# lpiccinelli-eth/UniDepth

Hardware: NVIDIA H100
Metric: images/sec UniDepthV2.infer ViT-L/14 480x640 (higher is better)
Workload: dtype f16 operands, f32 accumulate/residual

## Files before the change

unidepth_b200/csrc/attention.cu:

```cuda
#include "common.h"
#include "ptx.cuh"

namespace udb {

constexpr int AT_BQ = 128;
constexpr int AT_BK = 128;
constexpr int AT_STAGES = 3;
constexpr int AT_THREADS = 288;

struct AttnArgs {
  __half* out;
  int seq_q, seq_k, n_kv_tiles;
  int ldo, o_col0;
  int q_col0, k_col0, v_col0;
  float scale_log2;
};

__device__ __forceinline__ float ex2(float x) {
  float y;
  asm("ex2.approx.ftz.f32 %0, %1;" : "=f"(y) : "f"(x));
  return y;
}

template <int HD>
__global__ void __launch_bounds__(AT_THREADS, 1)
attn_fwd_kernel(const __grid_constant__ CUtensorMap tmQ, const __grid_constant__ CUtensorMap tmK,
                const __grid_constant__ CUtensorMap tmV, const AttnArgs p) {
  static_assert(HD == 64, "head_dim 64 only");
  constexpr int kQBytes = AT_BQ * HD * 2;
  constexpr int kKBytes = AT_BK * HD * 2;
  constexpr int NS = AT_STAGES;
  extern __shared__ __align__(1024) uint8_t smem[];
  uint8_t* sQ = smem;
  uint8_t* sK = sQ + kQBytes;
  uint8_t* sV = sK + NS * kKBytes;
  uint64_t* bars = reinterpret_cast<uint64_t*>(sV + NS * kKBytes);
  uint64_t* q_full = bars;
  uint64_t* k_full = bars + 1;
  uint64_t* v_full = k_full + NS;
  uint64_t* k_empty = v_full + NS;
  uint64_t* v_empty = k_empty + NS;

  const int warp = threadIdx.x >> 5;
  const int lane = threadIdx.x & 31;
  const int q0 = blockIdx.x * AT_BQ;
  const int head = blockIdx.y;
  const int b = blockIdx.z;
  const int n_tiles = p.n_kv_tiles;
  pdl_launch_dependents();

  if (threadIdx.x == 0) {
    if (smem_u32(smem) & 1023) __trap();
    prefetch_tmap(&tmQ);
    prefetch_tmap(&tmK);
    prefetch_tmap(&tmV);
    mbar_init(q_full, 1);
    for (int i = 0; i < NS; ++i) {
      mbar_init(&k_full[i], 1);
      mbar_init(&v_full[i], 1);
      mbar_init(&k_empty[i], 8);
      mbar_init(&v_empty[i], 8);
    }
    fence_barrier_init();
  }
  __syncthreads();
  pdl_wait();

  if (warp == 8) {
    const bool leader = elect_one();
    if (leader) {
      mbar_arrive_expect_tx(q_full, kQBytes);
      tma_load_3d(sQ, &tmQ, q_full, p.q_col0 + head * HD, q0, b);
    }
    __syncwarp();
    int st = 0;
    uint32_t ph = 1;
    for (int j = 0; j < n_tiles; ++j) {
      mbar_wait(&k_empty[st], ph);
      if (leader) {
        mbar_arrive_expect_tx(&k_full[st], kKBytes);
        tma_load_3d(sK + st * kKBytes, &tmK, &k_full[st], p.k_col0 + head * HD, j * AT_BK, b);
      }
      __syncwarp();
      mbar_wait(&v_empty[st], ph);
      if (leader) {
        mbar_arrive_expect_tx(&v_full[st], kKBytes);
        tma_load_3d(sV + st * kKBytes, &tmV, &v_full[st], p.v_col0 + head * HD, j * AT_BK, b);
      }
      __syncwarp();
      if (++st == NS) { st = 0; ph ^= 1; }
    }
    return;
  }

  const int wg = warp >> 2, wq = warp & 3;
  const int cq = 2 * (lane & 3);
  const float sc = p.scale_log2;
  const uint64_t dq = gmma_desc_sw128(smem_u32(sQ + wg * 64 * 128), 16, 1024);
  float o[HD / 2];
#pragma unroll
  for (int i = 0; i < HD / 2; ++i) o[i] = 0.f;
  float m_run[2] = {-INFINITY, -INFINITY}, l_run[2] = {0.f, 0.f};
  mbar_wait(q_full, 0);
  int st = 0;
  uint32_t ph = 0;
  for (int j = 0; j < n_tiles; ++j) {
    float s[AT_BK / 2];
    mbar_wait(&k_full[st], ph);
    {
      const uint64_t dk = gmma_desc_sw128(smem_u32(sK + st * kKBytes), 16, 1024);
      wgmma_fence();
#pragma unroll
      for (int k = 0; k < HD / 16; ++k) wgmma_ss_n128(s, dq + 2 * k, dk + 2 * k, k != 0 ? 1u : 0u);
      wgmma_commit();
      wgmma_wait<0>();
      wgmma_fence_regs(s);
    }
    if (lane == 0) mbar_arrive(&k_empty[st]);
    const int kv_left = p.seq_k - j * AT_BK;
    if (kv_left < AT_BK) {
#pragma unroll
      for (int i = 0; i < AT_BK / 2; ++i)
        if (8 * (i >> 2) + cq + (i & 1) >= kv_left) s[i] = -INFINITY;
    }
#pragma unroll
    for (int h = 0; h < 2; ++h) {
      float mx = -INFINITY;
#pragma unroll
      for (int jj = 0; jj < AT_BK / 8; ++jj) mx = fmaxf(mx, fmaxf(s[4 * jj + 2 * h], s[4 * jj + 2 * h + 1]));
      mx = fmaxf(mx, __shfl_xor_sync(0xffffffffu, mx, 1));
      mx = fmaxf(mx, __shfl_xor_sync(0xffffffffu, mx, 2));
      const float m_new = fmaxf(m_run[h], mx * sc);
      const float alpha = ex2(m_run[h] - m_new);
      m_run[h] = m_new;
      float ls = 0.f;
#pragma unroll
      for (int jj = 0; jj < AT_BK / 8; ++jj) {
        const float e0 = ex2(fmaf(s[4 * jj + 2 * h], sc, -m_new));
        const float e1 = ex2(fmaf(s[4 * jj + 2 * h + 1], sc, -m_new));
        s[4 * jj + 2 * h] = e0;
        s[4 * jj + 2 * h + 1] = e1;
        ls += e0 + e1;
      }
      l_run[h] = fmaf(l_run[h], alpha, ls);
#pragma unroll
      for (int jj = 0; jj < HD / 8; ++jj) {
        o[4 * jj + 2 * h] *= alpha;
        o[4 * jj + 2 * h + 1] *= alpha;
      }
    }
    uint32_t pa[AT_BK / 16][4];
#pragma unroll
    for (int kk = 0; kk < AT_BK / 16; ++kk)
#pragma unroll
      for (int r = 0; r < 4; ++r) pa[kk][r] = pack_half2(s[8 * kk + 2 * r], s[8 * kk + 2 * r + 1]);
    mbar_wait(&v_full[st], ph);
    {
      const uint64_t dv = gmma_desc_sw128(smem_u32(sV + st * kKBytes), 1024, 1024);
      wgmma_fence();
#pragma unroll
      for (int kk = 0; kk < AT_BK / 16; ++kk) wgmma_rs_n64_tb(o, pa[kk], dv + (uint64_t)(kk * 2048 >> 4), 1u);
      wgmma_commit();
      wgmma_wait<0>();
      wgmma_fence_regs(o);
    }
    if (lane == 0) mbar_arrive(&v_empty[st]);
    if (++st == NS) { st = 0; ph ^= 1; }
  }
#pragma unroll
  for (int h = 0; h < 2; ++h) {
    float l = l_run[h];
    l += __shfl_xor_sync(0xffffffffu, l, 1);
    l += __shfl_xor_sync(0xffffffffu, l, 2);
    const float inv = 1.0f / l;
    const int q = q0 + 64 * wg + 16 * wq + (lane >> 2) + 8 * h;
    if (q < p.seq_q) {
      __half* op = p.out + ((long long)b * p.seq_q + q) * p.ldo + p.o_col0 + head * HD + cq;
#pragma unroll
      for (int jj = 0; jj < HD / 8; ++jj)
        *reinterpret_cast<uint32_t*>(op + 8 * jj) = pack_half2(o[4 * jj + 2 * h] * inv, o[4 * jj + 2 * h + 1] * inv);
    }
  }
}

constexpr int SP_T = 64;
constexpr int SP_P = 65;
constexpr int SP_SMEM = (4 * SP_T * SP_P + 3 * SP_T) * 4;

__global__ void __launch_bounds__(256) attn_split_f32_kernel(const udb_attn_t a) {
  extern __shared__ float sp_smem[];
  float* Qs = sp_smem;
  float* Ks = Qs + SP_T * SP_P;
  float* Vs = Ks + SP_T * SP_P;
  float* Ps = Vs + SP_T * SP_P;
  float* m_s = Ps + SP_T * SP_P;
  float* l_s = m_s + SP_T;
  float* al_s = l_s + SP_T;
  const int t = threadIdx.x, ty = t >> 4, tx = t & 15;
  const int q0 = blockIdx.x * SP_T, h = blockIdx.y, b = blockIdx.z;
  const __half* qp = reinterpret_cast<const __half*>(a.q);
  const __half* kp = reinterpret_cast<const __half*>(a.k);
  const __half* vp = reinterpret_cast<const __half*>(a.v);
  auto ld = [](const __half* base, long long off, int lo_off) {
    return __half2float(base[off]) + (lo_off ? __half2float(base[off + lo_off]) : 0.f);
  };
  for (int i = t; i < SP_T * SP_T; i += 256) {
    const int r = i >> 6, d = i & 63;
    const int sq = q0 + r;
    Qs[r * SP_P + d] = sq < a.seq_q ? ld(qp, ((long long)b * a.seq_q + sq) * a.ldq + a.q_col0 + h * 64 + d, a.lo_off_q) * a.scale : 0.f;
  }
  if (t < SP_T) { m_s[t] = -INFINITY; l_s[t] = 0.f; }
  float O[4][4];
#pragma unroll
  for (int i = 0; i < 4; ++i)
#pragma unroll
    for (int j = 0; j < 4; ++j) O[i][j] = 0.f;
  const int n_kt = (a.seq_k + SP_T - 1) / SP_T;
  for (int kt = 0; kt < n_kt; ++kt) {
    __syncthreads();
    for (int i = t; i < SP_T * SP_T; i += 256) {
      const int r = i >> 6, d = i & 63;
      const int sk = kt * SP_T + r;
      const bool ok = sk < a.seq_k;
      const long long row = (long long)b * a.seq_k + sk;
      Ks[r * SP_P + d] = ok ? ld(kp, row * a.ldk + a.k_col0 + h * 64 + d, a.lo_off_k) : 0.f;
      Vs[r * SP_P + d] = ok ? ld(vp, row * a.ldv + a.v_col0 + h * 64 + d, a.lo_off_v) : 0.f;
    }
    __syncthreads();
    float S[4][4];
#pragma unroll
    for (int i = 0; i < 4; ++i)
#pragma unroll
      for (int j = 0; j < 4; ++j) S[i][j] = 0.f;
    for (int d = 0; d < 64; ++d) {
      float qv[4], kv[4];
#pragma unroll
      for (int i = 0; i < 4; ++i) qv[i] = Qs[(ty + 16 * i) * SP_P + d];
#pragma unroll
      for (int j = 0; j < 4; ++j) kv[j] = Ks[(tx + 16 * j) * SP_P + d];
#pragma unroll
      for (int i = 0; i < 4; ++i)
#pragma unroll
        for (int j = 0; j < 4; ++j) S[i][j] = fmaf(qv[i], kv[j], S[i][j]);
    }
#pragma unroll
    for (int i = 0; i < 4; ++i)
#pragma unroll
      for (int j = 0; j < 4; ++j) {
        const int c = tx + 16 * j;
        Ps[(ty + 16 * i) * SP_P + c] = (kt * SP_T + c < a.seq_k) ? S[i][j] : -INFINITY;
      }
    __syncthreads();
    {
      const int r = t >> 2, part = t & 3;
      float* pr = Ps + r * SP_P + part * 16;
      float mx = -INFINITY;
#pragma unroll
      for (int c = 0; c < 16; ++c) mx = fmaxf(mx, pr[c]);
      mx = fmaxf(mx, __shfl_xor_sync(0xffffffffu, mx, 1));
      mx = fmaxf(mx, __shfl_xor_sync(0xffffffffu, mx, 2));
      const float m_old = m_s[r];
      const float m_new = fmaxf(m_old, mx);
      float sum = 0.f;
#pragma unroll
      for (int c = 0; c < 16; ++c) {
        const float pv = expf(pr[c] - m_new);
        pr[c] = pv;
        sum += pv;
      }
      sum += __shfl_xor_sync(0xffffffffu, sum, 1);
      sum += __shfl_xor_sync(0xffffffffu, sum, 2);
      __syncwarp();
      if (part == 0) {
        const float al = expf(m_old - m_new);
        al_s[r] = al;
        m_s[r] = m_new;
        l_s[r] = l_s[r] * al + sum;
      }
    }
    __syncthreads();
#pragma unroll
    for (int i = 0; i < 4; ++i) {
      const float al = al_s[ty + 16 * i];
#pragma unroll
      for (int j = 0; j < 4; ++j) O[i][j] *= al;
    }
    for (int c = 0; c < SP_T; ++c) {
      float pv[4], vv[4];
#pragma unroll
      for (int i = 0; i < 4; ++i) pv[i] = Ps[(ty + 16 * i) * SP_P + c];
#pragma unroll
      for (int j = 0; j < 4; ++j) vv[j] = Vs[c * SP_P + tx + 16 * j];
#pragma unroll
      for (int i = 0; i < 4; ++i)
#pragma unroll
        for (int j = 0; j < 4; ++j) O[i][j] = fmaf(pv[i], vv[j], O[i][j]);
    }
  }
  __half* op = reinterpret_cast<__half*>(a.out);
#pragma unroll
  for (int i = 0; i < 4; ++i) {
    const int r = ty + 16 * i;
    const int sq = q0 + r;
    if (sq >= a.seq_q) continue;
    const float inv = 1.0f / l_s[r];
#pragma unroll
    for (int j = 0; j < 4; ++j) {
      const float v = O[i][j] * inv;
      const long long off = ((long long)b * a.seq_q + sq) * a.ldo + a.o_col0 + h * 64 + tx + 16 * j;
      const __half hi = __float2half_rn(v);
      op[off] = hi;
      if (a.lo_off_o) op[off + a.lo_off_o] = __float2half_rn(v - __half2float(hi));
    }
  }
}

}

extern "C" int udb_attention_f16(const udb_attn_t* a, void* stream) {
  using namespace udb;
  if (a->head_dim != 64) { set_error("udb_attention_f16: head_dim %d unsupported (64 only)", a->head_dim); return 1; }
  if ((a->ldq | a->ldk | a->ldv | a->ldo) % 8) { set_error("udb_attention_f16: leading dims must be multiples of 8"); return 1; }
  if (a->split) {
    static std::atomic<uint64_t> sp_mask{0};
    if (first_on_device(sp_mask)) {
      cudaError_t e = cudaFuncSetAttribute(attn_split_f32_kernel, cudaFuncAttributeMaxDynamicSharedMemorySize, SP_SMEM);
      if (e != cudaSuccess) { set_error("attention(split): cudaFuncSetAttribute: %s", cudaGetErrorString(e)); return 1; }
    }
    dim3 grid((a->seq_q + SP_T - 1) / SP_T, a->heads, a->B);
    attn_split_f32_kernel<<<grid, 256, SP_SMEM, reinterpret_cast<cudaStream_t>(stream)>>>(*a);
    return check_launch("attn_split_f32_kernel");
  }
  constexpr int HD = 64;
  CUtensorMap tq, tk, tv;
  const uint32_t box_q[3] = {HD, AT_BQ, 1};
  const uint32_t box_kv[3] = {HD, AT_BK, 1};
  {
    const uint64_t dims[3] = {(uint64_t)a->ldq, (uint64_t)a->seq_q, (uint64_t)a->B};
    const uint64_t str[2] = {(uint64_t)a->ldq * 2, (uint64_t)a->seq_q * a->ldq * 2};
    if (make_tmap_f16(&tq, a->q, 3, dims, str, box_q, true)) return 1;
  }
  {
    const uint64_t dims[3] = {(uint64_t)a->ldk, (uint64_t)a->seq_k, (uint64_t)a->B};
    const uint64_t str[2] = {(uint64_t)a->ldk * 2, (uint64_t)a->seq_k * a->ldk * 2};
    if (make_tmap_f16(&tk, a->k, 3, dims, str, box_kv, true)) return 1;
  }
  {
    const uint64_t dims[3] = {(uint64_t)a->ldv, (uint64_t)a->seq_k, (uint64_t)a->B};
    const uint64_t str[2] = {(uint64_t)a->ldv * 2, (uint64_t)a->seq_k * a->ldv * 2};
    if (make_tmap_f16(&tv, a->v, 3, dims, str, box_kv, true)) return 1;
  }
  AttnArgs p{};
  p.out = reinterpret_cast<__half*>(a->out);
  p.seq_q = a->seq_q; p.seq_k = a->seq_k;
  p.n_kv_tiles = (a->seq_k + AT_BK - 1) / AT_BK;
  p.ldo = a->ldo; p.o_col0 = a->o_col0;
  p.q_col0 = a->q_col0; p.k_col0 = a->k_col0; p.v_col0 = a->v_col0;
  p.scale_log2 = a->scale * 1.4426950408889634f;
  dim3 grid((a->seq_q + AT_BQ - 1) / AT_BQ, a->heads, a->B);
  note_work(4.0 * a->B * a->heads * (double)a->seq_q * a->seq_k * HD, 2.0 * a->B * a->heads * HD * (2.0 * a->seq_q + 2.0 * a->seq_k));
  constexpr int smem_bytes = 16384 + 2 * AT_STAGES * (AT_BK * 128) + 256;
  static std::atomic<uint64_t> attr_mask{0};
  if (first_on_device(attr_mask)) {
    cudaError_t ea = cudaFuncSetAttribute(attn_fwd_kernel<HD>, cudaFuncAttributeMaxDynamicSharedMemorySize, smem_bytes);
    if (ea != cudaSuccess) { set_error("attention: cudaFuncSetAttribute: %s", cudaGetErrorString(ea)); return 1; }
  }
  cudaError_t e = launch_ex(attn_fwd_kernel<HD>, grid, dim3(AT_THREADS), smem_bytes, reinterpret_cast<cudaStream_t>(stream), 1,
                            tq, tk, tv, p);
  if (e != cudaSuccess) { set_error("attn_fwd_kernel launch: %s", cudaGetErrorString(e)); return 1; }
  return check_launch("attn_fwd_kernel");
}
```

unidepth_b200/csrc/ptx.cuh:

```cuda
#pragma once
#include <cuda_fp16.h>
#include <cuda_runtime.h>
#include <stdint.h>
#include <stdio.h>

namespace udb {

__device__ __forceinline__ uint32_t smem_u32(const void* p) {
  return static_cast<uint32_t>(__cvta_generic_to_shared(p));
}

__device__ __forceinline__ bool elect_one() {
  uint32_t pred = 0;
  asm volatile(
      "{\n\t"
      ".reg .b32 rx;\n\t"
      ".reg .pred px;\n\t"
      "elect.sync rx|px, 0xffffffff;\n\t"
      "selp.b32 %0, 1, 0, px;\n\t"
      "}\n"
      : "=r"(pred));
  return pred != 0;
}

__device__ __forceinline__ void pdl_launch_dependents() {
  asm volatile("griddepcontrol.launch_dependents;" ::: "memory");
}
__device__ __forceinline__ void pdl_wait() { asm volatile("griddepcontrol.wait;" ::: "memory"); }

__device__ __forceinline__ void mbar_init(uint64_t* bar, uint32_t count) {
  asm volatile("mbarrier.init.shared::cta.b64 [%0], %1;" ::"r"(smem_u32(bar)), "r"(count));
}
__device__ __forceinline__ void fence_barrier_init() {
  asm volatile("fence.mbarrier_init.release.cluster;" ::: "memory");
}
__device__ __forceinline__ void mbar_arrive(uint64_t* bar) {
  asm volatile("mbarrier.arrive.shared::cta.b64 _, [%0];" ::"r"(smem_u32(bar)) : "memory");
}
__device__ __forceinline__ void mbar_arrive_expect_tx(uint64_t* bar, uint32_t bytes) {
  asm volatile("mbarrier.arrive.expect_tx.shared::cta.b64 _, [%0], %1;" ::"r"(smem_u32(bar)),
               "r"(bytes)
               : "memory");
}
__device__ __forceinline__ bool mbar_try_wait(uint64_t* bar, uint32_t parity) {
  uint32_t ok;
  asm volatile(
      "{\n\t"
      ".reg .pred p;\n\t"
      "mbarrier.try_wait.parity.shared::cta.b64 p, [%1], %2, %3;\n\t"
      "selp.b32 %0, 1, 0, p;\n\t"
      "}\n"
      : "=r"(ok)
      : "r"(smem_u32(bar)), "r"(parity), "r"(20000u)
      : "memory");
  return ok != 0;
}
#ifndef UDB_SPIN_LIMIT
#define UDB_SPIN_LIMIT (1u << 22)
#endif
__device__ __forceinline__ void mbar_wait(uint64_t* bar, uint32_t parity) {
  if (mbar_try_wait(bar, parity)) return;
  uint32_t spins = 0;
  while (!mbar_try_wait(bar, parity)) {
    if (++spins > UDB_SPIN_LIMIT) __trap();
  }
}

__device__ __forceinline__ void fence_proxy_async_smem() {
  asm volatile("fence.proxy.async.shared::cta;" ::: "memory");
}

__device__ __forceinline__ void prefetch_tmap(const void* tmap) {
  asm volatile("prefetch.tensormap [%0];" ::"l"(reinterpret_cast<uint64_t>(tmap)) : "memory");
}
__device__ __forceinline__ void tma_load_2d(void* smem_dst, const void* tmap, uint64_t* bar, int c0,
                                            int c1) {
  asm volatile(
      "cp.async.bulk.tensor.2d.shared::cluster.global.mbarrier::complete_tx::bytes"
      " [%0], [%1, {%3, %4}], [%2];" ::"r"(smem_u32(smem_dst)),
      "l"(reinterpret_cast<uint64_t>(tmap)), "r"(smem_u32(bar)), "r"(c0), "r"(c1)
      : "memory");
}
__device__ __forceinline__ void tma_load_3d(void* smem_dst, const void* tmap, uint64_t* bar, int c0,
                                            int c1, int c2) {
  asm volatile(
      "cp.async.bulk.tensor.3d.shared::cluster.global.mbarrier::complete_tx::bytes"
      " [%0], [%1, {%3, %4, %5}], [%2];" ::"r"(smem_u32(smem_dst)),
      "l"(reinterpret_cast<uint64_t>(tmap)), "r"(smem_u32(bar)), "r"(c0), "r"(c1), "r"(c2)
      : "memory");
}
__device__ __forceinline__ void tma_load_4d(void* smem_dst, const void* tmap, uint64_t* bar, int c0,
                                            int c1, int c2, int c3) {
  asm volatile(
      "cp.async.bulk.tensor.4d.shared::cluster.global.mbarrier::complete_tx::bytes"
      " [%0], [%1, {%3, %4, %5, %6}], [%2];" ::"r"(smem_u32(smem_dst)),
      "l"(reinterpret_cast<uint64_t>(tmap)), "r"(smem_u32(bar)), "r"(c0), "r"(c1), "r"(c2), "r"(c3)
      : "memory");
}


__device__ __forceinline__ void wgmma_fence() { asm volatile("wgmma.fence.sync.aligned;" ::: "memory"); }
__device__ __forceinline__ void wgmma_commit() { asm volatile("wgmma.commit_group.sync.aligned;" ::: "memory"); }
template <int N>
__device__ __forceinline__ void wgmma_wait() {
  asm volatile("wgmma.wait_group.sync.aligned %0;" ::"n"(N) : "memory");
}
template <int R>
__device__ __forceinline__ void wgmma_fence_regs(float (&d)[R]) {
#pragma unroll
  for (int i = 0; i < R; ++i) asm volatile("" : "+f"(d[i])::"memory");
}
template <uint32_t R>
__device__ __forceinline__ void setmaxnreg_inc() { asm volatile("setmaxnreg.inc.sync.aligned.u32 %0;" ::"n"(R)); }
template <uint32_t R>
__device__ __forceinline__ void setmaxnreg_dec() { asm volatile("setmaxnreg.dec.sync.aligned.u32 %0;" ::"n"(R)); }
__device__ __forceinline__ void bar_sync(int id, int threads) {
  asm volatile("bar.sync %0, %1;" ::"r"(id), "r"(threads) : "memory");
}

__device__ __forceinline__ uint64_t gmma_desc_sw128(uint32_t smem_addr, uint32_t lbo_bytes, uint32_t sbo_bytes) {
  uint64_t d = 0;
  d |= static_cast<uint64_t>((smem_addr & 0x3FFFF) >> 4);
  d |= static_cast<uint64_t>((lbo_bytes >> 4) & 0x3FFF) << 16;
  d |= static_cast<uint64_t>((sbo_bytes >> 4) & 0x3FFF) << 32;
  d |= static_cast<uint64_t>(1) << 62;
  return d;
}

__device__ __forceinline__ void wgmma_ss_n32(float (&d)[16], uint64_t da, uint64_t db, uint32_t scale_d) {
  asm volatile(
      "{\n\t.reg .pred p;\n\tsetp.ne.b32 p, %18, 0;\n\t"
      "wgmma.mma_async.sync.aligned.m64n32k16.f32.f16.f16 {%0, %1, %2, %3, %4, %5, %6, %7, %8, %9, %10, %11, %12, %13, %14, %15}, %16, %17, p, 1, 1, 0, 0;\n\t}\n"
      : "+f"(d[0]), "+f"(d[1]), "+f"(d[2]), "+f"(d[3]), "+f"(d[4]), "+f"(d[5]), "+f"(d[6]), "+f"(d[7]), "+f"(d[8]), "+f"(d[9]), "+f"(d[10]), "+f"(d[11]), "+f"(d[12]), "+f"(d[13]), "+f"(d[14]), "+f"(d[15])
      : "l"(da), "l"(db), "r"(scale_d));
}
__device__ __forceinline__ void wgmma_ss_n64(float (&d)[32], uint64_t da, uint64_t db, uint32_t scale_d) {
  asm volatile(
      "{\n\t.reg .pred p;\n\tsetp.ne.b32 p, %34, 0;\n\t"
      "wgmma.mma_async.sync.aligned.m64n64k16.f32.f16.f16 {%0, %1, %2, %3, %4, %5, %6, %7, %8, %9, %10, %11, %12, %13, %14, %15, %16, %17, %18, %19, %20, %21, %22, %23, %24, %25, %26, %27, %28, %29, %30, %31}, %32, %33, p, 1, 1, 0, 0;\n\t}\n"
      : "+f"(d[0]), "+f"(d[1]), "+f"(d[2]), "+f"(d[3]), "+f"(d[4]), "+f"(d[5]), "+f"(d[6]), "+f"(d[7]), "+f"(d[8]), "+f"(d[9]), "+f"(d[10]), "+f"(d[11]), "+f"(d[12]), "+f"(d[13]), "+f"(d[14]), "+f"(d[15]), "+f"(d[16]), "+f"(d[17]), "+f"(d[18]), "+f"(d[19]), "+f"(d[20]), "+f"(d[21]), "+f"(d[22]), "+f"(d[23]), "+f"(d[24]), "+f"(d[25]), "+f"(d[26]), "+f"(d[27]), "+f"(d[28]), "+f"(d[29]), "+f"(d[30]), "+f"(d[31])
      : "l"(da), "l"(db), "r"(scale_d));
}
__device__ __forceinline__ void wgmma_ss_n128(float (&d)[64], uint64_t da, uint64_t db, uint32_t scale_d) {
  asm volatile(
      "{\n\t.reg .pred p;\n\tsetp.ne.b32 p, %66, 0;\n\t"
      "wgmma.mma_async.sync.aligned.m64n128k16.f32.f16.f16 {%0, %1, %2, %3, %4, %5, %6, %7, %8, %9, %10, %11, %12, %13, %14, %15, %16, %17, %18, %19, %20, %21, %22, %23, %24, %25, %26, %27, %28, %29, %30, %31, %32, %33, %34, %35, %36, %37, %38, %39, %40, %41, %42, %43, %44, %45, %46, %47, %48, %49, %50, %51, %52, %53, %54, %55, %56, %57, %58, %59, %60, %61, %62, %63}, %64, %65, p, 1, 1, 0, 0;\n\t}\n"
      : "+f"(d[0]), "+f"(d[1]), "+f"(d[2]), "+f"(d[3]), "+f"(d[4]), "+f"(d[5]), "+f"(d[6]), "+f"(d[7]), "+f"(d[8]), "+f"(d[9]), "+f"(d[10]), "+f"(d[11]), "+f"(d[12]), "+f"(d[13]), "+f"(d[14]), "+f"(d[15]), "+f"(d[16]), "+f"(d[17]), "+f"(d[18]), "+f"(d[19]), "+f"(d[20]), "+f"(d[21]), "+f"(d[22]), "+f"(d[23]), "+f"(d[24]), "+f"(d[25]), "+f"(d[26]), "+f"(d[27]), "+f"(d[28]), "+f"(d[29]), "+f"(d[30]), "+f"(d[31]), "+f"(d[32]), "+f"(d[33]), "+f"(d[34]), "+f"(d[35]), "+f"(d[36]), "+f"(d[37]), "+f"(d[38]), "+f"(d[39]), "+f"(d[40]), "+f"(d[41]), "+f"(d[42]), "+f"(d[43]), "+f"(d[44]), "+f"(d[45]), "+f"(d[46]), "+f"(d[47]), "+f"(d[48]), "+f"(d[49]), "+f"(d[50]), "+f"(d[51]), "+f"(d[52]), "+f"(d[53]), "+f"(d[54]), "+f"(d[55]), "+f"(d[56]), "+f"(d[57]), "+f"(d[58]), "+f"(d[59]), "+f"(d[60]), "+f"(d[61]), "+f"(d[62]), "+f"(d[63])
      : "l"(da), "l"(db), "r"(scale_d));
}
__device__ __forceinline__ void wgmma_ss_n192(float (&d)[96], uint64_t da, uint64_t db, uint32_t scale_d) {
  asm volatile(
      "{\n\t.reg .pred p;\n\tsetp.ne.b32 p, %98, 0;\n\t"
      "wgmma.mma_async.sync.aligned.m64n192k16.f32.f16.f16 {%0, %1, %2, %3, %4, %5, %6, %7, %8, %9, %10, %11, %12, %13, %14, %15, %16, %17, %18, %19, %20, %21, %22, %23, %24, %25, %26, %27, %28, %29, %30, %31, %32, %33, %34, %35, %36, %37, %38, %39, %40, %41, %42, %43, %44, %45, %46, %47, %48, %49, %50, %51, %52, %53, %54, %55, %56, %57, %58, %59, %60, %61, %62, %63, %64, %65, %66, %67, %68, %69, %70, %71, %72, %73, %74, %75, %76, %77, %78, %79, %80, %81, %82, %83, %84, %85, %86, %87, %88, %89, %90, %91, %92, %93, %94, %95}, %96, %97, p, 1, 1, 0, 0;\n\t}\n"
      : "+f"(d[0]), "+f"(d[1]), "+f"(d[2]), "+f"(d[3]), "+f"(d[4]), "+f"(d[5]), "+f"(d[6]), "+f"(d[7]), "+f"(d[8]), "+f"(d[9]), "+f"(d[10]), "+f"(d[11]), "+f"(d[12]), "+f"(d[13]), "+f"(d[14]), "+f"(d[15]), "+f"(d[16]), "+f"(d[17]), "+f"(d[18]), "+f"(d[19]), "+f"(d[20]), "+f"(d[21]), "+f"(d[22]), "+f"(d[23]), "+f"(d[24]), "+f"(d[25]), "+f"(d[26]), "+f"(d[27]), "+f"(d[28]), "+f"(d[29]), "+f"(d[30]), "+f"(d[31]), "+f"(d[32]), "+f"(d[33]), "+f"(d[34]), "+f"(d[35]), "+f"(d[36]), "+f"(d[37]), "+f"(d[38]), "+f"(d[39]), "+f"(d[40]), "+f"(d[41]), "+f"(d[42]), "+f"(d[43]), "+f"(d[44]), "+f"(d[45]), "+f"(d[46]), "+f"(d[47]), "+f"(d[48]), "+f"(d[49]), "+f"(d[50]), "+f"(d[51]), "+f"(d[52]), "+f"(d[53]), "+f"(d[54]), "+f"(d[55]), "+f"(d[56]), "+f"(d[57]), "+f"(d[58]), "+f"(d[59]), "+f"(d[60]), "+f"(d[61]), "+f"(d[62]), "+f"(d[63]), "+f"(d[64]), "+f"(d[65]), "+f"(d[66]), "+f"(d[67]), "+f"(d[68]), "+f"(d[69]), "+f"(d[70]), "+f"(d[71]), "+f"(d[72]), "+f"(d[73]), "+f"(d[74]), "+f"(d[75]), "+f"(d[76]), "+f"(d[77]), "+f"(d[78]), "+f"(d[79]), "+f"(d[80]), "+f"(d[81]), "+f"(d[82]), "+f"(d[83]), "+f"(d[84]), "+f"(d[85]), "+f"(d[86]), "+f"(d[87]), "+f"(d[88]), "+f"(d[89]), "+f"(d[90]), "+f"(d[91]), "+f"(d[92]), "+f"(d[93]), "+f"(d[94]), "+f"(d[95])
      : "l"(da), "l"(db), "r"(scale_d));
}
__device__ __forceinline__ void wgmma_ss_n256(float (&d)[128], uint64_t da, uint64_t db, uint32_t scale_d) {
  asm volatile(
      "{\n\t.reg .pred p;\n\tsetp.ne.b32 p, %130, 0;\n\t"
      "wgmma.mma_async.sync.aligned.m64n256k16.f32.f16.f16 {%0, %1, %2, %3, %4, %5, %6, %7, %8, %9, %10, %11, %12, %13, %14, %15, %16, %17, %18, %19, %20, %21, %22, %23, %24, %25, %26, %27, %28, %29, %30, %31, %32, %33, %34, %35, %36, %37, %38, %39, %40, %41, %42, %43, %44, %45, %46, %47, %48, %49, %50, %51, %52, %53, %54, %55, %56, %57, %58, %59, %60, %61, %62, %63, %64, %65, %66, %67, %68, %69, %70, %71, %72, %73, %74, %75, %76, %77, %78, %79, %80, %81, %82, %83, %84, %85, %86, %87, %88, %89, %90, %91, %92, %93, %94, %95, %96, %97, %98, %99, %100, %101, %102, %103, %104, %105, %106, %107, %108, %109, %110, %111, %112, %113, %114, %115, %116, %117, %118, %119, %120, %121, %122, %123, %124, %125, %126, %127}, %128, %129, p, 1, 1, 0, 0;\n\t}\n"
      : "+f"(d[0]), "+f"(d[1]), "+f"(d[2]), "+f"(d[3]), "+f"(d[4]), "+f"(d[5]), "+f"(d[6]), "+f"(d[7]), "+f"(d[8]), "+f"(d[9]), "+f"(d[10]), "+f"(d[11]), "+f"(d[12]), "+f"(d[13]), "+f"(d[14]), "+f"(d[15]), "+f"(d[16]), "+f"(d[17]), "+f"(d[18]), "+f"(d[19]), "+f"(d[20]), "+f"(d[21]), "+f"(d[22]), "+f"(d[23]), "+f"(d[24]), "+f"(d[25]), "+f"(d[26]), "+f"(d[27]), "+f"(d[28]), "+f"(d[29]), "+f"(d[30]), "+f"(d[31]), "+f"(d[32]), "+f"(d[33]), "+f"(d[34]), "+f"(d[35]), "+f"(d[36]), "+f"(d[37]), "+f"(d[38]), "+f"(d[39]), "+f"(d[40]), "+f"(d[41]), "+f"(d[42]), "+f"(d[43]), "+f"(d[44]), "+f"(d[45]), "+f"(d[46]), "+f"(d[47]), "+f"(d[48]), "+f"(d[49]), "+f"(d[50]), "+f"(d[51]), "+f"(d[52]), "+f"(d[53]), "+f"(d[54]), "+f"(d[55]), "+f"(d[56]), "+f"(d[57]), "+f"(d[58]), "+f"(d[59]), "+f"(d[60]), "+f"(d[61]), "+f"(d[62]), "+f"(d[63]), "+f"(d[64]), "+f"(d[65]), "+f"(d[66]), "+f"(d[67]), "+f"(d[68]), "+f"(d[69]), "+f"(d[70]), "+f"(d[71]), "+f"(d[72]), "+f"(d[73]), "+f"(d[74]), "+f"(d[75]), "+f"(d[76]), "+f"(d[77]), "+f"(d[78]), "+f"(d[79]), "+f"(d[80]), "+f"(d[81]), "+f"(d[82]), "+f"(d[83]), "+f"(d[84]), "+f"(d[85]), "+f"(d[86]), "+f"(d[87]), "+f"(d[88]), "+f"(d[89]), "+f"(d[90]), "+f"(d[91]), "+f"(d[92]), "+f"(d[93]), "+f"(d[94]), "+f"(d[95]), "+f"(d[96]), "+f"(d[97]), "+f"(d[98]), "+f"(d[99]), "+f"(d[100]), "+f"(d[101]), "+f"(d[102]), "+f"(d[103]), "+f"(d[104]), "+f"(d[105]), "+f"(d[106]), "+f"(d[107]), "+f"(d[108]), "+f"(d[109]), "+f"(d[110]), "+f"(d[111]), "+f"(d[112]), "+f"(d[113]), "+f"(d[114]), "+f"(d[115]), "+f"(d[116]), "+f"(d[117]), "+f"(d[118]), "+f"(d[119]), "+f"(d[120]), "+f"(d[121]), "+f"(d[122]), "+f"(d[123]), "+f"(d[124]), "+f"(d[125]), "+f"(d[126]), "+f"(d[127])
      : "l"(da), "l"(db), "r"(scale_d));
}
__device__ __forceinline__ void wgmma_rs_n64_tb(float (&d)[32], const uint32_t (&a)[4], uint64_t db, uint32_t scale_d) {
  asm volatile(
      "{\n\t.reg .pred p;\n\tsetp.ne.b32 p, %37, 0;\n\t"
      "wgmma.mma_async.sync.aligned.m64n64k16.f32.f16.f16 {%0, %1, %2, %3, %4, %5, %6, %7, %8, %9, %10, %11, %12, %13, %14, %15, %16, %17, %18, %19, %20, %21, %22, %23, %24, %25, %26, %27, %28, %29, %30, %31}, {%32, %33, %34, %35}, %36, p, 1, 1, 1;\n\t}\n"
      : "+f"(d[0]), "+f"(d[1]), "+f"(d[2]), "+f"(d[3]), "+f"(d[4]), "+f"(d[5]), "+f"(d[6]), "+f"(d[7]), "+f"(d[8]), "+f"(d[9]), "+f"(d[10]), "+f"(d[11]), "+f"(d[12]), "+f"(d[13]), "+f"(d[14]), "+f"(d[15]), "+f"(d[16]), "+f"(d[17]), "+f"(d[18]), "+f"(d[19]), "+f"(d[20]), "+f"(d[21]), "+f"(d[22]), "+f"(d[23]), "+f"(d[24]), "+f"(d[25]), "+f"(d[26]), "+f"(d[27]), "+f"(d[28]), "+f"(d[29]), "+f"(d[30]), "+f"(d[31])
      : "r"(a[0]), "r"(a[1]), "r"(a[2]), "r"(a[3]), "l"(db), "r"(scale_d));
}

template <int N> struct WgmmaSS;
template <> struct WgmmaSS<32> { static __device__ __forceinline__ void run(float (&d)[16], uint64_t a, uint64_t b, uint32_t s) { wgmma_ss_n32(d, a, b, s); } };
template <> struct WgmmaSS<64> { static __device__ __forceinline__ void run(float (&d)[32], uint64_t a, uint64_t b, uint32_t s) { wgmma_ss_n64(d, a, b, s); } };
template <> struct WgmmaSS<128> { static __device__ __forceinline__ void run(float (&d)[64], uint64_t a, uint64_t b, uint32_t s) { wgmma_ss_n128(d, a, b, s); } };
template <> struct WgmmaSS<192> { static __device__ __forceinline__ void run(float (&d)[96], uint64_t a, uint64_t b, uint32_t s) { wgmma_ss_n192(d, a, b, s); } };
template <> struct WgmmaSS<256> { static __device__ __forceinline__ void run(float (&d)[128], uint64_t a, uint64_t b, uint32_t s) { wgmma_ss_n256(d, a, b, s); } };

__device__ __forceinline__ uint64_t pack2(float lo, float hi) {
  uint64_t d;
  asm("mov.b64 %0, {%1, %2};" : "=l"(d) : "f"(lo), "f"(hi));
  return d;
}
__device__ __forceinline__ uint64_t pack2u(uint32_t lo, uint32_t hi) {
  uint64_t d;
  asm("mov.b64 %0, {%1, %2};" : "=l"(d) : "r"(lo), "r"(hi));
  return d;
}
__device__ __forceinline__ void unpack2(uint64_t v, float& lo, float& hi) {
  asm("mov.b64 {%0, %1}, %2;" : "=f"(lo), "=f"(hi) : "l"(v));
}
__device__ __forceinline__ uint64_t fma2(uint64_t a, uint64_t b, uint64_t c) {
  float a0, a1, b0, b1, c0, c1;
  unpack2(a, a0, a1);
  unpack2(b, b0, b1);
  unpack2(c, c0, c1);
  return pack2(fmaf(a0, b0, c0), fmaf(a1, b1, c1));
}
__device__ __forceinline__ uint64_t mul2(uint64_t a, uint64_t b) {
  float a0, a1, b0, b1;
  unpack2(a, a0, a1);
  unpack2(b, b0, b1);
  return pack2(__fmul_rn(a0, b0), __fmul_rn(a1, b1));
}

__device__ __forceinline__ float gelu_erf(float x) {
  return 0.5f * x * (1.0f + erff(x * 0.70710678118654752440f));
}
__device__ __forceinline__ float gelu_erf_fast(float x) {
  const float z = fabsf(x) * 0.70710678118654752440f;
  float t;
  asm("rcp.approx.ftz.f32 %0, %1;" : "=f"(t) : "f"(fmaf(0.3275911f, z, 1.0f)));
  float poly = fmaf(t, 1.061405429f, -1.453152027f);
  poly = fmaf(poly, t, 1.421413741f);
  poly = fmaf(poly, t, -0.284496736f);
  poly = fmaf(poly, t, 0.254829592f);
  poly *= t;
  float e;
  asm("ex2.approx.ftz.f32 %0, %1;" : "=f"(e) : "f"(z * z * -1.4426950408889634f));
  const float erf_abs = fmaf(-poly, e, 1.0f);
  const float h = 0.5f * x;
  return fmaf(copysignf(erf_abs, x), h, h);
}
__device__ __forceinline__ void gelu_erf_pair(float& x0, float& x1) {
  const float z0 = fabsf(x0) * 0.70710678118654752440f, z1 = fabsf(x1) * 0.70710678118654752440f;
  const uint64_t z = pack2(z0, z1);
  uint64_t q = fma2(z, pack2(0.0000430638f, 0.0000430638f), pack2(0.0002765672f, 0.0002765672f));
  q = fma2(q, z, pack2(0.0001520143f, 0.0001520143f));
  q = fma2(q, z, pack2(0.0092705272f, 0.0092705272f));
  q = fma2(q, z, pack2(0.0422820123f, 0.0422820123f));
  q = fma2(q, z, pack2(0.0705230784f, 0.0705230784f));
  q = fma2(q, z, pack2(1.0f, 1.0f));
  q = mul2(q, q);
  q = mul2(q, q);
  q = mul2(q, q);
  q = mul2(q, q);
  float p0, p1, r0, r1;
  unpack2(q, p0, p1);
  asm("rcp.approx.ftz.f32 %0, %1;" : "=f"(r0) : "f"(p0));
  asm("rcp.approx.ftz.f32 %0, %1;" : "=f"(r1) : "f"(p1));
  const float h0 = 0.5f * x0, h1 = 0.5f * x1;
  x0 = fmaf(copysignf(1.0f - r0, x0), h0, h0);
  x1 = fmaf(copysignf(1.0f - r1, x1), h1, h1);
}
__device__ __forceinline__ float leaky(float x) { return x > 0.f ? x : 0.01f * x; }

__device__ __forceinline__ uint32_t pack_half2(float a, float b) {
  __half2 h = __floats2half2_rn(a, b);
  return *reinterpret_cast<uint32_t*>(&h);
}

}
```

Before: 211.3.

## Overlap QK and PV wgmma across tiles with ping-pong warpgroup scheduling

Restructures the attention consumer loop FA3-style. The QK^T GEMM for tile j and the PV GEMM for tile j-1 are issued together, and softmax runs while the PV GEMM is still in flight. Named barriers alternate the two consumer warpgroups so one issues tensor-core work while the other does softmax. This hides the exp/softmax latency behind wgmma, at the cost of more live registers for s/pa/o and more complex synchronisation.

```diff
diff --git a/unidepth_b200/csrc/attention.cu b/unidepth_b200/csrc/attention.cu
--- a/unidepth_b200/csrc/attention.cu
+++ b/unidepth_b200/csrc/attention.cu
@@ -100,23 +100,24 @@
   float o[HD / 2];
 #pragma unroll
   for (int i = 0; i < HD / 2; ++i) o[i] = 0.f;
+  float s[AT_BK / 2];
+  uint32_t pa[AT_BK / 16][4];
   float m_run[2] = {-INFINITY, -INFINITY}, l_run[2] = {0.f, 0.f};
-  mbar_wait(q_full, 0);
-  int st = 0;
-  uint32_t ph = 0;
-  for (int j = 0; j < n_tiles; ++j) {
-    float s[AT_BK / 2];
-    mbar_wait(&k_full[st], ph);
-    {
-      const uint64_t dk = gmma_desc_sw128(smem_u32(sK + st * kKBytes), 16, 1024);
-      wgmma_fence();
-#pragma unroll
-      for (int k = 0; k < HD / 16; ++k) wgmma_ss_n128(s, dq + 2 * k, dk + 2 * k, k != 0 ? 1u : 0u);
-      wgmma_commit();
-      wgmma_wait<0>();
-      wgmma_fence_regs(s);
-    }
-    if (lane == 0) mbar_arrive(&k_empty[st]);
+  float alpha[2];
+
+  auto issue_qk = [&](int st) {
+    const uint64_t dk = gmma_desc_sw128(smem_u32(sK + st * kKBytes), 16, 1024);
+#pragma unroll
+    for (int k = 0; k < HD / 16; ++k) wgmma_ss_n128(s, dq + 2 * k, dk + 2 * k, k != 0 ? 1u : 0u);
+    wgmma_commit();
+  };
+  auto issue_pv = [&](int st) {
+    const uint64_t dv = gmma_desc_sw128(smem_u32(sV + st * kKBytes), 1024, 1024);
+#pragma unroll
+    for (int kk = 0; kk < AT_BK / 16; ++kk) wgmma_rs_n64_tb(o, pa[kk], dv + (uint64_t)(kk * 2048 >> 4), 1u);
+    wgmma_commit();
+  };
+  auto softmax = [&](int j) {
     const int kv_left = p.seq_k - j * AT_BK;
     if (kv_left < AT_BK) {
 #pragma unroll
@@ -131,7 +132,7 @@
       mx = fmaxf(mx, __shfl_xor_sync(0xffffffffu, mx, 1));
       mx = fmaxf(mx, __shfl_xor_sync(0xffffffffu, mx, 2));
       const float m_new = fmaxf(m_run[h], mx * sc);
-      const float alpha = ex2(m_run[h] - m_new);
+      alpha[h] = ex2(m_run[h] - m_new);
       m_run[h] = m_new;
       float ls = 0.f;
 #pragma unroll
@@ -142,31 +143,66 @@
         s[4 * jj + 2 * h + 1] = e1;
         ls += e0 + e1;
       }
-      l_run[h] = fmaf(l_run[h], alpha, ls);
+      l_run[h] = fmaf(l_run[h], alpha[h], ls);
+    }
+  };
+  auto rescale_and_pack = [&]() {
+#pragma unroll
+    for (int h = 0; h < 2; ++h)
 #pragma unroll
       for (int jj = 0; jj < HD / 8; ++jj) {
-        o[4 * jj + 2 * h] *= alpha;
-        o[4 * jj + 2 * h + 1] *= alpha;
-      }
-    }
-    uint32_t pa[AT_BK / 16][4];
+        o[4 * jj + 2 * h] *= alpha[h];
+        o[4 * jj + 2 * h + 1] *= alpha[h];
+      }
 #pragma unroll
     for (int kk = 0; kk < AT_BK / 16; ++kk)
 #pragma unroll
       for (int r = 0; r < 4; ++r) pa[kk][r] = pack_half2(s[8 * kk + 2 * r], s[8 * kk + 2 * r + 1]);
-    mbar_wait(&v_full[st], ph);
-    {
-      const uint64_t dv = gmma_desc_sw128(smem_u32(sV + st * kKBytes), 1024, 1024);
-      wgmma_fence();
-#pragma unroll
-      for (int kk = 0; kk < AT_BK / 16; ++kk) wgmma_rs_n64_tb(o, pa[kk], dv + (uint64_t)(kk * 2048 >> 4), 1u);
-      wgmma_commit();
-      wgmma_wait<0>();
-      wgmma_fence_regs(o);
-    }
-    if (lane == 0) mbar_arrive(&v_empty[st]);
-    if (++st == NS) { st = 0; ph ^= 1; }
-  }
+  };
+  const int my_turn = 1 + wg, other_turn = 2 - wg;
+  mbar_wait(q_full, 0);
+  if (wg == 1) bar_arrive(other_turn, 256);
+  int kst = 0, vst = 0;
+  uint32_t kph = 0, vph = 0;
+
+  mbar_wait(&k_full[kst], kph);
+  bar_sync(my_turn, 256);
+  wgmma_fence();
+  issue_qk(kst);
+  bar_arrive(other_turn, 256);
+  wgmma_wait<0>();
+  wgmma_fence_regs(s);
+  if (lane == 0) mbar_arrive(&k_empty[kst]);
+  if (++kst == NS) { kst = 0; kph ^= 1; }
+  softmax(0);
+  rescale_and_pack();
+  for (int j = 1; j < n_tiles; ++j) {
+    mbar_wait(&k_full[kst], kph);
+    mbar_wait(&v_full[vst], vph);
+    bar_sync(my_turn, 256);
+    wgmma_fence();
+    issue_qk(kst);
+    issue_pv(vst);
+    bar_arrive(other_turn, 256);
+    wgmma_wait<1>();
+    wgmma_fence_regs(s);
+    if (lane == 0) mbar_arrive(&k_empty[kst]);
+    if (++kst == NS) { kst = 0; kph ^= 1; }
+    softmax(j);
+    wgmma_wait<0>();
+    wgmma_fence_regs(o);
+    wgmma_fence_regs(pa);
+    if (lane == 0) mbar_arrive(&v_empty[vst]);
+    if (++vst == NS) { vst = 0; vph ^= 1; }
+    rescale_and_pack();
+  }
+  mbar_wait(&v_full[vst], vph);
+  bar_sync(my_turn, 256);
+  wgmma_fence();
+  issue_pv(vst);
+  if (wg == 0) bar_arrive(other_turn, 256);
+  wgmma_wait<0>();
+  wgmma_fence_regs(o);
 #pragma unroll
   for (int h = 0; h < 2; ++h) {
     float l = l_run[h];
diff --git a/unidepth_b200/csrc/ptx.cuh b/unidepth_b200/csrc/ptx.cuh
--- a/unidepth_b200/csrc/ptx.cuh
+++ b/unidepth_b200/csrc/ptx.cuh
@@ -110,12 +110,22 @@
 #pragma unroll
   for (int i = 0; i < R; ++i) asm volatile("" : "+f"(d[i])::"memory");
 }
+template <int R, int C>
+__device__ __forceinline__ void wgmma_fence_regs(uint32_t (&a)[R][C]) {
+#pragma unroll
+  for (int i = 0; i < R; ++i)
+#pragma unroll
+    for (int j = 0; j < C; ++j) asm volatile("" : "+r"(a[i][j])::"memory");
+}
 template <uint32_t R>
 __device__ __forceinline__ void setmaxnreg_inc() { asm volatile("setmaxnreg.inc.sync.aligned.u32 %0;" ::"n"(R)); }
 template <uint32_t R>
 __device__ __forceinline__ void setmaxnreg_dec() { asm volatile("setmaxnreg.dec.sync.aligned.u32 %0;" ::"n"(R)); }
 __device__ __forceinline__ void bar_sync(int id, int threads) {
   asm volatile("bar.sync %0, %1;" ::"r"(id), "r"(threads) : "memory");
+}
+__device__ __forceinline__ void bar_arrive(int id, int threads) {
+  asm volatile("bar.arrive %0, %1;" ::"r"(id), "r"(threads) : "memory");
 }
 
 __device__ __forceinline__ uint64_t gmma_desc_sw128(uint32_t smem_addr, uint32_t lbo_bytes, uint32_t sbo_bytes) {
```

After: 213.7 (median of 6 runs). 1.01x the previous value.
